# DarlingHang/st-nerf

Measured on NVIDIA H100. Metric: rays/sec, higher is better.
Workload: dtype f32 via fp16x3 split products (wgmma), f32 accumulate

## Files before the change

st-nerf_b200/csrc/mlp_tc.cu:

```cuda
#include <cuda_fp16.h>
#include <string.h>
#include <type_traits>
#include <vector>
#include "mlp_tc.cuh"
#include "resample.cuh"

namespace stnerf {

namespace {

constexpr int TILE_M = 128;
constexpr int ABLOCK = 16384;
constexpr int STAGE_BYTES = 16384;
constexpr int NTHREADS = 384;
constexpr int MATH_WG0 = 1, N_MATH_WARPS = 8;
constexpr int MAX_STAGE = 8;
constexpr int REGS_WG0 = 56, REGS_MATH = 224;
static_assert(128 * REGS_WG0 + 256 * REGS_MATH <= 384 * 168, "register file");
constexpr int BAR_WFULL = 0, BAR_WEMPTY = 8, BAR_RAWFULL = 16, BAR_RAWEMPTY = 18;
constexpr int MISC_ROWS = 256;
constexpr int MISC_PART = MISC_ROWS + 128 * 24;
constexpr int MISC_CDF = MISC_PART + 2048;
constexpr int MISC_TOTAL = MISC_CDF + 512;

__device__ __forceinline__ uint32_t smem_u32(const void* p) { return (uint32_t)__cvta_generic_to_shared(p); }

__device__ __forceinline__ void mbar_init(uint32_t bar, uint32_t count) {
  asm volatile("mbarrier.init.shared::cta.b64 [%0], %1;" ::"r"(bar), "r"(count) : "memory");
}
__device__ __forceinline__ void mbar_arrive(uint32_t bar) {
  asm volatile("mbarrier.arrive.shared::cta.b64 _, [%0];" ::"r"(bar) : "memory");
}
__device__ __forceinline__ void mbar_arrive_if(uint32_t bar, bool pred) {
  asm volatile("{\n\t.reg .pred p;\n\tsetp.ne.b32 p, %1, 0;\n\t@p mbarrier.arrive.shared::cta.b64 _, [%0];\n\t}" ::"r"(bar), "r"((uint32_t)pred)
               : "memory");
}
__device__ __forceinline__ void mbar_expect_tx(uint32_t bar, uint32_t bytes) {
  asm volatile("mbarrier.arrive.expect_tx.shared::cta.b64 _, [%0], %1;" ::"r"(bar), "r"(bytes) : "memory");
}
__device__ __forceinline__ void mbar_wait(uint32_t bar, uint32_t parity) {
  asm volatile(
      "{\n\t.reg .pred p;\n\t.reg .u32 c;\n\t"
      "mov.u32 c, 0;\n"
      "WAIT_%=:\n\t"
      "mbarrier.try_wait.parity.shared::cta.b64 p, [%0], %1;\n\t"
      "@p bra.uni DONE_%=;\n\t"
      "add.u32 c, c, 1;\n\t"
      "setp.gt.u32 p, c, 67108864;\n\t"
      "@p trap;\n\t"
      "bra.uni WAIT_%=;\n"
      "DONE_%=:\n\t}" ::"r"(bar), "r"(parity)
      : "memory");
}
__device__ __forceinline__ void bulk_g2s(uint32_t dst, const void* src, uint32_t bytes, uint32_t bar) {
  asm volatile("cp.async.bulk.shared::cluster.global.mbarrier::complete_tx::bytes [%0], [%1], %2, [%3];" ::"r"(dst),
               "l"(src), "r"(bytes), "r"(bar)
               : "memory");
}
__device__ __forceinline__ void fence_proxy_async() { asm volatile("fence.proxy.async.shared::cta;" ::: "memory"); }
template <int R>
__device__ __forceinline__ void setmaxnreg_dec() { asm volatile("setmaxnreg.dec.sync.aligned.u32 %0;" ::"n"(R)); }
template <int R>
__device__ __forceinline__ void setmaxnreg_inc() { asm volatile("setmaxnreg.inc.sync.aligned.u32 %0;" ::"n"(R)); }
__device__ __forceinline__ void wg_bar_sync(int wg) { asm volatile("bar.sync %0, 128;" ::"r"(1 + wg) : "memory"); }

__device__ __forceinline__ void load_stage_elect(uint32_t dst, const void* src, uint32_t bytes, uint32_t bar) {
  asm volatile(
      "{\n\t.reg .pred pe;\n\t"
      "elect.sync _|pe, 0xffffffff;\n\t"
      "@pe mbarrier.arrive.expect_tx.shared::cta.b64 _, [%3], %2;\n\t"
      "@pe cp.async.bulk.shared::cluster.global.mbarrier::complete_tx::bytes [%0], [%1], %2, [%3];\n\t}" ::"r"(dst),
      "l"(src), "r"(bytes), "r"(bar)
      : "memory");
}

__device__ __forceinline__ uint64_t desc_sw128(uint32_t saddr) {
  return (uint64_t)((saddr >> 4) & 0x3FFF) | ((uint64_t)1 << 16) | ((uint64_t)(1024 >> 4) << 32) | ((uint64_t)1 << 62);
}
__device__ __forceinline__ uint64_t desc_sw64(uint32_t saddr) {
  return (uint64_t)((saddr >> 4) & 0x3FFF) | ((uint64_t)1 << 16) | ((uint64_t)(512 >> 4) << 32) | ((uint64_t)2 << 62);
}
__device__ __forceinline__ void wgmma_fence() { asm volatile("wgmma.fence.sync.aligned;" ::: "memory"); }
__device__ __forceinline__ void wgmma_commit() { asm volatile("wgmma.commit_group.sync.aligned;" ::: "memory"); }
template <int N>
__device__ __forceinline__ void wgmma_wait() { asm volatile("wgmma.wait_group.sync.aligned %0;" ::"n"(N) : "memory"); }
template <int R>
__device__ __forceinline__ void acc_fence(float (&d)[128]) {
#pragma unroll
  for (int i = 0; i < R; ++i) asm volatile("" : "+f"(d[i])::"memory");
}

#define WGMMA_D_LO "%0, %1, %2, %3, %4, %5, %6, %7, %8, %9, %10, %11, %12, %13, %14, %15, %16, %17, %18, %19, %20, %21, %22, %23, %24, %25, %26, %27, %28, %29, %30, %31, %32, %33, %34, %35, %36, %37, %38, %39, %40, %41, %42, %43, %44, %45, %46, %47, %48, %49, %50, %51, %52, %53, %54, %55, %56, %57, %58, %59, %60, %61, %62, %63"
#define WGMMA_D_HI "%64, %65, %66, %67, %68, %69, %70, %71, %72, %73, %74, %75, %76, %77, %78, %79, %80, %81, %82, %83, %84, %85, %86, %87, %88, %89, %90, %91, %92, %93, %94, %95, %96, %97, %98, %99, %100, %101, %102, %103, %104, %105, %106, %107, %108, %109, %110, %111, %112, %113, %114, %115, %116, %117, %118, %119, %120, %121, %122, %123, %124, %125, %126, %127"
#define WGMMA_OPS_LO(d) \
    "+f"(d[0]), "+f"(d[1]), "+f"(d[2]), "+f"(d[3]), "+f"(d[4]), "+f"(d[5]), "+f"(d[6]), "+f"(d[7]), \
    "+f"(d[8]), "+f"(d[9]), "+f"(d[10]), "+f"(d[11]), "+f"(d[12]), "+f"(d[13]), "+f"(d[14]), "+f"(d[15]), \
    "+f"(d[16]), "+f"(d[17]), "+f"(d[18]), "+f"(d[19]), "+f"(d[20]), "+f"(d[21]), "+f"(d[22]), "+f"(d[23]), \
    "+f"(d[24]), "+f"(d[25]), "+f"(d[26]), "+f"(d[27]), "+f"(d[28]), "+f"(d[29]), "+f"(d[30]), "+f"(d[31]), \
    "+f"(d[32]), "+f"(d[33]), "+f"(d[34]), "+f"(d[35]), "+f"(d[36]), "+f"(d[37]), "+f"(d[38]), "+f"(d[39]), \
    "+f"(d[40]), "+f"(d[41]), "+f"(d[42]), "+f"(d[43]), "+f"(d[44]), "+f"(d[45]), "+f"(d[46]), "+f"(d[47]), \
    "+f"(d[48]), "+f"(d[49]), "+f"(d[50]), "+f"(d[51]), "+f"(d[52]), "+f"(d[53]), "+f"(d[54]), "+f"(d[55]), \
    "+f"(d[56]), "+f"(d[57]), "+f"(d[58]), "+f"(d[59]), "+f"(d[60]), "+f"(d[61]), "+f"(d[62]), "+f"(d[63])
#define WGMMA_OPS_HI(d) \
    "+f"(d[64]), "+f"(d[65]), "+f"(d[66]), "+f"(d[67]), "+f"(d[68]), "+f"(d[69]), "+f"(d[70]), "+f"(d[71]), \
    "+f"(d[72]), "+f"(d[73]), "+f"(d[74]), "+f"(d[75]), "+f"(d[76]), "+f"(d[77]), "+f"(d[78]), "+f"(d[79]), \
    "+f"(d[80]), "+f"(d[81]), "+f"(d[82]), "+f"(d[83]), "+f"(d[84]), "+f"(d[85]), "+f"(d[86]), "+f"(d[87]), \
    "+f"(d[88]), "+f"(d[89]), "+f"(d[90]), "+f"(d[91]), "+f"(d[92]), "+f"(d[93]), "+f"(d[94]), "+f"(d[95]), \
    "+f"(d[96]), "+f"(d[97]), "+f"(d[98]), "+f"(d[99]), "+f"(d[100]), "+f"(d[101]), "+f"(d[102]), "+f"(d[103]), \
    "+f"(d[104]), "+f"(d[105]), "+f"(d[106]), "+f"(d[107]), "+f"(d[108]), "+f"(d[109]), "+f"(d[110]), "+f"(d[111]), \
    "+f"(d[112]), "+f"(d[113]), "+f"(d[114]), "+f"(d[115]), "+f"(d[116]), "+f"(d[117]), "+f"(d[118]), "+f"(d[119]), \
    "+f"(d[120]), "+f"(d[121]), "+f"(d[122]), "+f"(d[123]), "+f"(d[124]), "+f"(d[125]), "+f"(d[126]), "+f"(d[127])

__device__ __forceinline__ void wgmma_n256(float (&d)[128], uint64_t da, uint64_t db) {
  asm volatile(
      "{\n\t.reg .pred p;\n\tsetp.ne.b32 p, %130, 0;\n\t"
      "wgmma.mma_async.sync.aligned.m64n256k16.f32.f16.f16 "
      "{" WGMMA_D_LO ", " WGMMA_D_HI "}, %128, %129, p, 1, 1, 0, 0;\n\t}"
      : WGMMA_OPS_LO(d), WGMMA_OPS_HI(d)
      : "l"(da), "l"(db), "r"(1));
}
__device__ __forceinline__ void wgmma_n128(float (&d)[128], uint64_t da, uint64_t db) {
  asm volatile(
      "{\n\t.reg .pred p;\n\tsetp.ne.b32 p, %66, 0;\n\t"
      "wgmma.mma_async.sync.aligned.m64n128k16.f32.f16.f16 "
      "{" WGMMA_D_LO "}, %64, %65, p, 1, 1, 0, 0;\n\t}"
      : WGMMA_OPS_LO(d)
      : "l"(da), "l"(db), "r"(1));
}
__device__ __forceinline__ void wgmma_n256_rs(float (&d)[128], const uint32_t* a, uint64_t db) {
  asm volatile(
      "{\n\t.reg .pred p;\n\tsetp.ne.b32 p, %133, 0;\n\t"
      "wgmma.mma_async.sync.aligned.m64n256k16.f32.f16.f16 "
      "{" WGMMA_D_LO ", " WGMMA_D_HI "}, {%128, %129, %130, %131}, %132, p, 1, 1, 0;\n\t}"
      : WGMMA_OPS_LO(d), WGMMA_OPS_HI(d)
      : "r"(a[0]), "r"(a[1]), "r"(a[2]), "r"(a[3]), "l"(db), "r"(1));
}
__device__ __forceinline__ void wgmma_n128_rs(float (&d)[128], const uint32_t* a, uint64_t db) {
  asm volatile(
      "{\n\t.reg .pred p;\n\tsetp.ne.b32 p, %69, 0;\n\t"
      "wgmma.mma_async.sync.aligned.m64n128k16.f32.f16.f16 "
      "{" WGMMA_D_LO "}, {%64, %65, %66, %67}, %68, p, 1, 1, 0;\n\t}"
      : WGMMA_OPS_LO(d)
      : "r"(a[0]), "r"(a[1]), "r"(a[2]), "r"(a[3]), "l"(db), "r"(1));
}

template <int N>
__device__ __forceinline__ void wgmma_k16(float (&d)[128], uint64_t da, uint64_t db) {
  if (N == 256) wgmma_n256(d, da, db);
  else wgmma_n128(d, da, db);
}
template <int N>
__device__ __forceinline__ void wgmma_k16_rs(float (&d)[128], const uint32_t* a, uint64_t db) {
  if (N == 256) wgmma_n256_rs(d, a, db);
  else wgmma_n128_rs(d, a, db);
}

__device__ __forceinline__ uint32_t pack_f16x2(float a, float b) {
  uint32_t r;
  asm("cvt.rn.satfinite.f16x2.f32 %0, %1, %2;" : "=r"(r) : "f"(b), "f"(a));
  return r;
}
__device__ __forceinline__ float2 unpack_f16x2(uint32_t p) {
  return __half22float2(*reinterpret_cast<const __half2*>(&p));
}

__host__ __device__ inline uint32_t sw128_offset(int row, int col) {
  return (uint32_t)((row >> 3) * 1024 + (row & 7) * 128 + ((((col >> 3) ^ (row & 7)) & 7) << 4) + ((col & 7) << 1));
}
__host__ __device__ inline uint32_t sw64_offset(int row, int col) {
  return (uint32_t)((row >> 3) * 512 + (row & 7) * 64 + ((((col >> 3) ^ ((row >> 1) & 3)) & 3) << 4) + ((col & 7) << 1));
}

enum { NET_SPACE = 0, NET_MOTION = 1 };

template <int NET> struct Sched;
template <> struct Sched<NET_SPACE> {
  static constexpr int N_LAYERS = 8;
  static constexpr bool lo_in_regs = true;
  static constexpr int act_base = 0, enc_base = 4 * ABLOCK;
  static constexpr int ENC_LO_STRIDE = ABLOCK;
  static constexpr int n_stage = 7, stage_bytes = STAGE_BYTES;
  static constexpr int ring_base = 6 * ABLOCK, misc_base = ring_base + n_stage * stage_bytes, smem_total = misc_base + MISC_TOTAL;
  static_assert(smem_total <= 232448, "shared memory budget (227 KB per CTA)");
  __host__ __device__ static constexpr int n_out(int l) { return l == 7 ? 128 : 256; }
  __host__ __device__ static constexpr int act_chunks(int l) { return l == 0 ? 0 : 4; }
  __host__ __device__ static constexpr int enc_chunks(int l) { return (l == 0 || l == 4) ? 1 : 0; }
  __host__ __device__ static constexpr bool enc_first(int l) { return l == 4; }
};
template <> struct Sched<NET_MOTION> {
  static constexpr int N_LAYERS = 5;
  static constexpr bool lo_in_regs = false;
  static constexpr int act_base = 0, enc_base = 0;
  static constexpr int LO_STRIDE = 2 * ABLOCK;
  static constexpr int ENC_LO_STRIDE = 2 * ABLOCK;
  static constexpr int n_stage = 8, stage_bytes = 8192;
  static constexpr int ring_base = 4 * ABLOCK, misc_base = ring_base + n_stage * stage_bytes, smem_total = misc_base + MISC_TOTAL;
  __host__ __device__ static constexpr int n_out(int) { return 128; }
  __host__ __device__ static constexpr int act_chunks(int l) { return l == 0 ? 0 : 2; }
  __host__ __device__ static constexpr int enc_chunks(int l) { return l == 0 ? 2 : 0; }
  __host__ __device__ static constexpr bool enc_first(int) { return false; }
};
static_assert(Sched<NET_SPACE>::n_stage <= MAX_STAGE && Sched<NET_MOTION>::n_stage <= MAX_STAGE, "barrier slots");

enum { A_HI = 0, A_LO = 1, A_HI_LO = 2 };
template <int A>
struct WStep {
  static constexpr int a = A;
  uint32_t offset;
  uint32_t sub;
};
template <int NET>
struct WSched {
  using S = Sched<NET>;
  __host__ __device__ static constexpr int n_chunks(int l) { return S::act_chunks(l) + S::enc_chunks(l); }
  __host__ __device__ static constexpr uint32_t stage_bytes(int l) { return (uint32_t)S::n_out(l) * 64; }
  __host__ __device__ static constexpr size_t layer_bytes(int l) { return (size_t)n_chunks(l) * 2  * 2  * stage_bytes(l); }
  __host__ __device__ static constexpr int chunk_at(int l, int c) {
    return S::enc_first(l) ? (c == 0 ? S::act_chunks(l) : c - 1) : c;
  }
  static constexpr bool enc_first_valid() {
    for (int l = 0; l < S::N_LAYERS; ++l)
      if (S::enc_first(l) && (S::act_chunks(l) == 0 || S::enc_chunks(l) == 0)) return false;
    return true;
  }
  static_assert(enc_first_valid(), "enc_first(l) needs activation chunks and an encoding chunk to reorder");
  template <bool LOFIRST, class C, class F>
  __device__ __forceinline__ static void for_each_step(int l, bool split, C&& chunk, F&& f) {
    const int nact = S::act_chunks(l), nch = nact + S::enc_chunks(l);
    const uint32_t bytes = stage_bytes(l);
    auto at = [&](const auto& a, int c, uint32_t sub, uint32_t lo_stage, auto op) {
      f(a, WStep<decltype(op)::value>{(2 * (2 * (uint32_t)c + sub) + lo_stage) * bytes, sub});
    };
    using HI = std::integral_constant<int, A_HI>;
    using LO = std::integral_constant<int, A_LO>;
    using HI_LO = std::integral_constant<int, A_HI_LO>;
    if (!LOFIRST || !split) {
      for (int c = 0; c < nch; ++c) {
        const auto a = chunk(chunk_at(l, c));
        for (uint32_t sub = 0; sub < 2; ++sub) {
          if (split) { at(a, c, sub, 1u, HI()); at(a, c, sub, 0u, HI_LO()); }
          else at(a, c, sub, 0u, HI());
        }
      }
    } else {
      for (int c = 0; c < nch; ++c) {
        const auto a = chunk(chunk_at(l, c));
        for (uint32_t sub = 0; sub < 2; ++sub) { at(a, c, sub, 1u, HI()); at(a, c, sub, 0u, LO()); }
      }
      for (int c = 0; c < nch; ++c) {
        const auto a = chunk(chunk_at(l, c));
        for (uint32_t sub = 0; sub < 2; ++sub) at(a, c, sub, 0u, HI());
      }
    }
  }
};

template <int NET>
__host__ __device__ constexpr size_t stream_bytes_per_tile() {
  size_t n = 0;
  for (int l = 0; l < Sched<NET>::N_LAYERS; ++l) n += WSched<NET>::layer_bytes(l);
  return n;
}

struct TcParams {
  FuseCoarse fuse;
  PointSrc src;
  const uint8_t* wstream;
  const float* aux;
  const float* cbuf;
  int exact;
  int single_last;
  int lo_first;
  float* raw;
  float* rgb_out;
  float* sigma_out;
  float* xyz_out;
  float* flow_out;
  const int* lerp_flag;
  int lerp_force;
};

constexpr int AUX_BIAS = 0, AUX_WSIG = 8 * 256, AUX_BSIG = AUX_WSIG + 256, AUX_WOUT = AUX_BSIG + 4,
              AUX_BOUT = AUX_WOUT + 3 * 128, AUX_FLOATS = AUX_BOUT + 4;


struct Pt { float x, y, z, tm; int out_index; int cidx; };

__device__ __forceinline__ Pt fetch_pt(const PointSrc& s, long long p, long long n_points) {
  Pt q;
  q.x = q.y = q.z = q.tm = 0.f;
  q.out_index = -1;
  q.cidx = 0;
  if (p >= n_points) return q;
  if (s.mode == SRC_EXPLICIT) {
    const float* pp = s.pos + p * s.pos_stride;
    q.x = pp[0]; q.y = pp[1]; q.z = pp[2];
    if (s.times) q.tm = s.times[p * s.time_stride];
    q.out_index = (int)p;
    q.cidx = (int)p;
    return q;
  }
  const long long slot = p / s.S;
  const int k = (int)(p - slot * s.S);
  const long long ray = s.hit ? (long long)s.hit[slot] : slot;
  const float* rp = s.rays + ray * s.ray_stride;
  q.tm = rp[6 + s.layer];
  q.out_index = (int)(ray * s.S + k);
  q.cidx = (int)slot;
  if (s.mode == SRC_XYZ) {
    q.x = s.pos[3 * p]; q.y = s.pos[3 * p + 1]; q.z = s.pos[3 * p + 2];
    return q;
  }
  if (s.mode == SRC_XYZ_MAP) {
    const int m = s.src_map[ray * s.S + k];
    const float* pp = (m < s.n_first) ? s.pos + 3 * (slot * s.n_first + m) : s.pos2 + 3 * (slot * (s.S - s.n_first) + (m - s.n_first));
    q.x = pp[0]; q.y = pp[1]; q.z = pp[2];
    return q;
  }
  const float tt = s.t[ray * s.S + k];
  float v[3] = {__fadd_rn(__fmul_rn(tt, rp[3]), rp[0]), __fadd_rn(__fmul_rn(tt, rp[4]), rp[1]),
                __fadd_rn(__fmul_rn(tt, rp[5]), rp[2])};
#pragma unroll
  for (int a = 0; a < 3; ++a) {
    if (s.shift_on) v[a] = __fsub_rn(v[a], s.shift[a]);
    if (s.scale_on) v[a] = __fadd_rn(__fdiv_rn(__fsub_rn(v[a], s.pivot[a]), s.scale), s.pivot[a]);
  }
  q.x = v[0]; q.y = v[1]; q.z = v[2];
  return q;
}

struct SinCos3 { float s0, s1, s2, c0, c1, c2; };
struct SinCos4 { float s0, s1, s2, s3, c0, c1, c2, c3; };
__device__ __noinline__ SinCos3 sincos_full3(float x0, float x1, float x2) {
  SinCos3 r;
  sincosf(x0, &r.s0, &r.c0); sincosf(x1, &r.s1, &r.c1); sincosf(x2, &r.s2, &r.c2);
  return r;
}
__device__ __noinline__ SinCos4 sincos_full4(float x0, float x1, float x2, float x3) {
  SinCos4 r;
  sincosf(x0, &r.s0, &r.c0); sincosf(x1, &r.s1, &r.c1); sincosf(x2, &r.s2, &r.c2); sincosf(x3, &r.s3, &r.c3);
  return r;
}

template <int NV>
__device__ __forceinline__ void store_row_split(uint8_t* hi_blk, int lo_stride, int row, int col0, const float (&v)[NV],
                                                bool exact) {
#pragma unroll
  for (int g = 0; g < NV / 8; ++g) {
    uint32_t hp[4], lp[4];
#pragma unroll
    for (int e = 0; e < 4; ++e) {
      const float a = v[g * 8 + 2 * e], b = v[g * 8 + 2 * e + 1];
      hp[e] = pack_f16x2(a, b);
      const float2 hf = unpack_f16x2(hp[e]);
      lp[e] = pack_f16x2(a - hf.x, b - hf.y);
    }
    const uint32_t off = sw128_offset(row, col0 + g * 8);
    *reinterpret_cast<uint4*>(hi_blk + off) = make_uint4(hp[0], hp[1], hp[2], hp[3]);
    if (exact) *reinterpret_cast<uint4*>(hi_blk + lo_stride + off) = make_uint4(lp[0], lp[1], lp[2], lp[3]);
  }
}

template <int half, int piece>
__device__ __forceinline__ void encode_space_piece(uint8_t* smem, const Pt& pt, int row, bool exact, float (&carry)[2]) {
  using S = Sched<NET_SPACE>;
  uint8_t* enc = smem + S::enc_base;
  const float xs[3] = {pt.x, pt.y, pt.z};
  float v[16];
  auto trig = [&](int f, float* dst) {
    const float fr = (float)(1 << f);
    const SinCos3 q = sincos_full3(xs[0] * fr, xs[1] * fr, xs[2] * fr);
    dst[0] = q.s0; dst[1] = q.s1; dst[2] = q.s2; dst[3] = q.c0; dst[4] = q.c1; dst[5] = q.c2;
  };
  if (piece == 0) {
    float t3[6];
    trig(5 * half + 0, v); trig(5 * half + 1, v + 6); trig(5 * half + 2, t3);
    v[12] = t3[0]; v[13] = t3[1]; v[14] = t3[2]; v[15] = t3[3];
    carry[0] = t3[4]; carry[1] = t3[5];
  } else {
    v[0] = carry[0]; v[1] = carry[1];
    trig(5 * half + 3, v + 2); trig(5 * half + 4, v + 8);
    v[14] = half == 0 ? xs[0] : xs[2];
    v[15] = half == 0 ? xs[1] : 0.f;
  }
  store_row_split<16>(enc, S::ENC_LO_STRIDE, row, half * 32 + piece * 16, v, exact);
}

template <int half, int piece>
__device__ __forceinline__ void encode_motion_piece(uint8_t* smem, const Pt& pt, int row, bool exact, bool lerp) {
  using S = Sched<NET_MOTION>;
  uint8_t* enc = smem + S::enc_base + half * ABLOCK;
  const float lo_t = floorf(pt.tm), wgt = pt.tm - lo_t, omw = 1.0f - wgt;
  const float in4[4] = {pt.x, pt.y, pt.z, pt.tm};
  auto trig = [&](int f, float* dst) {
    const float fr = (float)(1 << f);
    if (!lerp) {
      const SinCos4 q = sincos_full4(in4[0] * fr, in4[1] * fr, in4[2] * fr, in4[3] * fr);
      dst[0] = q.s0; dst[1] = q.s1; dst[2] = q.s2; dst[3] = q.s3; dst[4] = q.c0; dst[5] = q.c1; dst[6] = q.c2; dst[7] = q.c3;
    } else {
      const SinCos4 q = sincos_full4(in4[0] * fr, in4[1] * fr, in4[2] * fr, lo_t * fr);
      const SinCos3 q1 = sincos_full3((lo_t + 1.0f) * fr, 0.f, 0.f);
      const float s0[4] = {q.s0, q.s1, q.s2, q.s3}, c0[4] = {q.c0, q.c1, q.c2, q.c3};
      const float s1[4] = {q.s0, q.s1, q.s2, q1.s0}, c1[4] = {q.c0, q.c1, q.c2, q1.c0};
#pragma unroll
      for (int d = 0; d < 4; ++d) {
        dst[d] = __fadd_rn(__fmul_rn(omw, s0[d]), __fmul_rn(wgt, s1[d]));
        dst[4 + d] = __fadd_rn(__fmul_rn(omw, c0[d]), __fmul_rn(wgt, c1[d]));
      }
    }
  };
  float v[16];
  trig(5 * half + 2 * piece, v);
  if (piece < 2) {
    trig(5 * half + 2 * piece + 1, v + 8);
  } else {
#pragma unroll
    for (int d = 0; d < 4; ++d) {
      float a = 0.f;
      if (half == 0) {
        a = in4[d];
        if (lerp) {
          const float lo = d < 3 ? in4[d] : lo_t, hi = d < 3 ? in4[d] : lo_t + 1.0f;
          a = __fadd_rn(__fmul_rn(omw, lo), __fmul_rn(wgt, hi));
        }
      }
      v[8 + d] = a; v[12 + d] = 0.f;
    }
  }
  store_row_split<16>(enc, S::ENC_LO_STRIDE, row, piece * 16, v, exact);
}

template <int NET, int piece>
__device__ __forceinline__ void encode_piece(uint8_t* smem, const Pt& pt, int row, int half, bool exact, bool lerp,
                                             float (&carry)[2]) {
  if (NET == NET_SPACE) {
    if (half == 0) encode_space_piece<0, piece < 2 ? piece : 1>(smem, pt, row, exact, carry);
    else encode_space_piece<1, piece < 2 ? piece : 1>(smem, pt, row, exact, carry);
  } else {
    if (half == 0) encode_motion_piece<0, piece>(smem, pt, row, exact, lerp);
    else encode_motion_piece<1, piece>(smem, pt, row, exact, lerp);
  }
}

template <int NZ>
__device__ __noinline__ void fused_composite_loop(const TcParams& P, const float* rows, float* cdf, uint32_t bar_full, uint32_t bar_empty,
                                                  long long n_tiles, int j, int lane) {
  const FuseCoarse& F = P.fuse;
  const PointSrc& src = P.src;
  const long long n_slots = src.count ? (long long)(*src.count) : src.n_slots;
  const int n1 = 64, n2 = F.n2;
  uint32_t n = 0;
  for (long long tile = blockIdx.x; tile < n_tiles; tile += gridDim.x, ++n) {
    mbar_wait(bar_full, n & 1);
    const long long slot = tile * 2 + j;
    if (slot < n_slots) {
      const long long ray = src.hit ? (long long)src.hit[slot] : slot;
      const float* tp = src.t + ray * n1;
      const float4* rp = reinterpret_cast<const float4*>(rows) + j * 64;
      float t[2], sg[2];
#pragma unroll
      for (int s = 0; s < 2; ++s) {
        const int k = s * 32 + lane;
        const float tk = __ldg(tp + k);
        float v = rp[k].w;
        if (F.is_bkgd) {
          if (tk < F.near_plane) v = 0.0f;
        } else {
          if (tk < 0.0f) v = 0.0f;
          if (F.apply_thr && v < F.thr) v = 0.0f;
        }
        t[s] = tk;
        sg[s] = v;
      }
      const float* up = F.u ? F.u + ray * n2 : nullptr;
      const uint64_t seed = F.seed;
      const uint32_t stream = 64u + (uint32_t)F.layer;
      const unsigned long long gid = F.idmap(F.ray_base + ray);
      rs::LayerOut lo;
      rs::composite_resample_ray<2, NZ>(
          t, sg, n1, n2, F.boarder,
          [rp, lane](int s) {
            const float4 v = rp[s * 32 + lane];
            return make_float3(__fdiv_rn(1.0f, __fadd_rn(1.0f, expf(-v.x))), __fdiv_rn(1.0f, __fadd_rn(1.0f, expf(-v.y))),
                               __fdiv_rn(1.0f, __fadd_rn(1.0f, expf(-v.z))));
          },
          [up, seed, stream, gid](int jj) { return up ? up[jj] : philox_uniform(seed, stream, gid, (uint32_t)jj); },
          cdf, F.t_fine + ray * (n1 + n2), lane, lo, F.z_new ? F.z_new + ray * n2 : nullptr,
          F.z_new ? F.src_map + ray * (n1 + n2) : nullptr);
      if (F.img && lane < 5) {
        const long long rg = F.ray_base + ray;
        const float v = lane == 0 ? lo.pix[0] : lane == 1 ? lo.pix[1] : lane == 2 ? lo.pix[2] : lane == 3 ? lo.pix[3] : lo.pix[4];
        if (F.pixels) F.img[rg * 5 + lane] = v;
        else if (lane < 3) F.img[rg * 3 + lane] = v;
        else F.img[(long long)lane * F.n_total + rg] = v;
      }
    }
    __syncwarp();
    if (lane == 0) mbar_arrive(bar_empty);
  }
}

template <int NET, int N, bool LOFIRST>
__device__ __forceinline__ void mma_layer(float (&acc)[128], const uint32_t (&alo)[64], int l, bool sp, uint32_t sbase,
                                          uint32_t a_row, uint32_t bars, uint32_t& cnt, int lane) {
  using S = Sched<NET>;
  using W = WSched<NET>;
  constexpr uint32_t NST = S::n_stage;
#pragma unroll
  for (int i = 0; i < N / 2; ++i) acc[i] = 0.f;
  acc_fence<N / 2>(acc);
  wgmma_fence();
  const int nact = S::act_chunks(l);
  int pend = -1;
  auto release = [&](int s) {
    __syncwarp();
    mbar_arrive_if(bars + 8u * (uint32_t)(BAR_WEMPTY + s), lane == 0);
  };
  auto a_block = [&](int ch) {
    uint32_t hi, lo = 0;
    int z = -1;
    if (ch < nact) {
      hi = sbase + S::act_base + ch * ABLOCK + a_row;
      if constexpr (S::lo_in_regs) z = ch;
      else lo = hi + S::LO_STRIDE;
    } else {
      hi = sbase + S::enc_base + (ch - nact) * ABLOCK + a_row;
      lo = hi + S::ENC_LO_STRIDE;
    }
    return make_int3((int)hi, (int)lo, z);
  };
  W::template for_each_step<LOFIRST>(l, sp, a_block, [&](const int3& a, auto st) {
    const uint32_t hi = (uint32_t)a.x + 64u * st.sub, lo = (uint32_t)a.y + 64u * st.sub;
    const uint32_t s = cnt % NST, n = cnt / NST;
    mbar_wait(bars + 8u * (BAR_WFULL + s), n & 1);
    const uint32_t w = sbase + S::ring_base + s * S::stage_bytes;
    auto mma_lo = [&]() {
      if (S::lo_in_regs && a.z >= 0) {
        const int q = 2 * a.z + (int)st.sub;
#pragma unroll
        for (int i = 0; i < 8; ++i)
          if (q == i) {
#pragma unroll
            for (int ks = 0; ks < 2; ++ks) wgmma_k16_rs<N>(acc, &alo[8 * i + 4 * ks], desc_sw64(w + ks * 32));
          }
      } else {
#pragma unroll
        for (int ks = 0; ks < 2; ++ks) wgmma_k16<N>(acc, desc_sw128(lo + ks * 32), desc_sw64(w + ks * 32));
      }
    };
    if constexpr (decltype(st)::a == A_LO) {
      mma_lo();
    } else {
#pragma unroll
      for (int ks = 0; ks < 2; ++ks) wgmma_k16<N>(acc, desc_sw128(hi + ks * 32), desc_sw64(w + ks * 32));
      if constexpr (decltype(st)::a == A_HI_LO) mma_lo();
    }
    wgmma_commit();
    wgmma_wait<1>();
    if (pend >= 0) release(pend);
    pend = (int)s;
    ++cnt;
  });
  wgmma_wait<0>();
  acc_fence<N / 2>(acc);
  release(pend);
}

template <int NET, int N, bool SIGMA>
__device__ __forceinline__ void epi_hidden(const float (&acc)[128], const float* __restrict__ bias, const float* __restrict__ wsig,
                                           uint8_t* smem, int r0, int cq, bool lo_too, float& sig0, float& sig1,
                                           uint32_t (&alo)[64]) {
  using S = Sched<NET>;
#pragma unroll
  for (int j = 0; j < N / 8; ++j) {
    const int col = 8 * j + cq;
    const float2 b = __ldg(reinterpret_cast<const float2*>(bias + col));
    const float v00 = fmaxf(acc[4 * j] + b.x, 0.f), v01 = fmaxf(acc[4 * j + 1] + b.y, 0.f);
    const float v10 = fmaxf(acc[4 * j + 2] + b.x, 0.f), v11 = fmaxf(acc[4 * j + 3] + b.y, 0.f);
    if (SIGMA) {
      const float2 w = __ldg(reinterpret_cast<const float2*>(wsig + col));
      sig0 = fmaf(v00, w.x, sig0); sig0 = fmaf(v01, w.y, sig0);
      sig1 = fmaf(v10, w.x, sig1); sig1 = fmaf(v11, w.y, sig1);
    }
    uint8_t* blk = smem + S::act_base + (col >> 6) * ABLOCK;
    const uint32_t o0 = sw128_offset(r0, col & 63), o1 = sw128_offset(r0 + 8, col & 63);
    const uint32_t h0 = pack_f16x2(v00, v01), h1 = pack_f16x2(v10, v11);
    *reinterpret_cast<uint32_t*>(blk + o0) = h0;
    *reinterpret_cast<uint32_t*>(blk + o1) = h1;
    const float2 f0 = unpack_f16x2(h0), f1 = unpack_f16x2(h1);
    const uint32_t l0 = pack_f16x2(v00 - f0.x, v01 - f0.y), l1 = pack_f16x2(v10 - f1.x, v11 - f1.y);
    if constexpr (S::lo_in_regs) {
      alo[2 * j] = l0;
      alo[2 * j + 1] = l1;
    } else if (lo_too) {
      *reinterpret_cast<uint32_t*>(blk + S::LO_STRIDE + o0) = l0;
      *reinterpret_cast<uint32_t*>(blk + S::LO_STRIDE + o1) = l1;
    }
  }
}

__device__ __forceinline__ float quad_sum(float v) {
  v += __shfl_xor_sync(0xffffffffu, v, 1);
  v += __shfl_xor_sync(0xffffffffu, v, 2);
  return v;
}

template <int NET, bool LOFIRST>
__global__ void __launch_bounds__(NTHREADS, 1) mlp_tc_kernel(const __grid_constant__ TcParams P) {
  using S = Sched<NET>;
  extern __shared__ __align__(1024) uint8_t smem[];
  const uint32_t sbase = smem_u32(smem);
  if ((sbase & 1023u) != 0) {
    if (threadIdx.x == 0) printf("stnerf mlp_tc: dynamic shared memory base %u is not 1024-byte aligned\n", sbase);
    __trap();
  }
  const uint32_t bars = sbase + S::misc_base;
  auto BAR = [bars](int i) { return bars + 8u * (uint32_t)i; };
  Pt* s_rows = reinterpret_cast<Pt*>(smem + S::misc_base + MISC_ROWS);
  float* s_part = reinterpret_cast<float*>(smem + S::misc_base + MISC_PART);

  const int tid = threadIdx.x, lane = tid & 31;
  const int warp = __shfl_sync(0xffffffffu, tid >> 5, 0);
  const int wgi = __shfl_sync(0xffffffffu, tid >> 7, 0);
  const bool exact = P.exact != 0;
  const bool single_last = P.single_last != 0;
  auto split = [&](int l) { return exact && !(single_last && l == S::N_LAYERS - 1); };
  const long long n_points = src_num_points(P.src);
  const long long n_tiles = (n_points + TILE_M - 1) / TILE_M;
  constexpr uint32_t NST = S::n_stage;
  if (tid == 0) {
    for (int i = 0; i < MAX_STAGE; ++i) { mbar_init(BAR(BAR_WFULL + i), 1); mbar_init(BAR(BAR_WEMPTY + i), N_MATH_WARPS); }
    for (int j = 0; j < 2; ++j) {
      mbar_init(BAR(BAR_RAWFULL + j), 4);
      mbar_init(BAR(BAR_RAWEMPTY + j), 1);
    }
    asm volatile("fence.mbarrier_init.release.cluster;" ::: "memory");
  }
  __syncthreads();

  if (wgi < MATH_WG0) {
    if constexpr (S::lo_in_regs) setmaxnreg_dec<REGS_WG0>();
    if (warp == 0) {
      using W = WSched<NET>;
      uint32_t cnt = 0;
      for (long long tile = blockIdx.x; tile < n_tiles; tile += gridDim.x) {
        const uint8_t* layer = P.wstream;
        for (int l = 0; l < S::N_LAYERS; ++l) {
          W::template for_each_step<LOFIRST>(l, split(l), [](int) { return 0; }, [&](int, auto st) {
            const uint32_t s = cnt % NST, n = cnt / NST;
            mbar_wait(BAR(BAR_WEMPTY + s), (n & 1) ^ 1);
            load_stage_elect(sbase + S::ring_base + s * S::stage_bytes, layer + st.offset, W::stage_bytes(l), BAR(BAR_WFULL + s));
            ++cnt;
          });
          layer += W::layer_bytes(l);
        }
      }
    } else if (NET == NET_SPACE && (warp == 2 || warp == 3)) {
      if (P.fuse.on) {
        const int j = warp - 2;
        float* cdf = reinterpret_cast<float*>(smem + S::misc_base + MISC_CDF) + j * 64;
        if (P.fuse.n2 <= 128)
          fused_composite_loop<4>(P, s_part, cdf, BAR(BAR_RAWFULL + j), BAR(BAR_RAWEMPTY + j), n_tiles, j, lane);
        else
          fused_composite_loop<8>(P, s_part, cdf, BAR(BAR_RAWFULL + j), BAR(BAR_RAWEMPTY + j), n_tiles, j, lane);
      }
    }
  } else {
    if constexpr (S::lo_in_regs) setmaxnreg_inc<REGS_MATH>();
    const int wg = wgi - MATH_WG0;
    const int wt = tid & 127;
    const int erow = wg * 64 + (wt & 63), ehalf = wt >> 6;
    const int r0 = wg * 64 + (wt >> 5) * 16 + (lane >> 2);
    const int cq = 2 * (lane & 3);
    const uint32_t a_row = (uint32_t)wg * 8u * 1024u;
    const float* bias_all = P.aux + AUX_BIAS;
    const bool lerp = (NET == NET_MOTION) && (P.lerp_force >= 0 ? (P.lerp_force != 0) : (P.lerp_flag && *P.lerp_flag != 0));
    const bool fused = (NET == NET_SPACE) && P.fuse.on;
    uint32_t cnt = 0, tile_no = 0;
    float acc[128];
    uint32_t alo[64];
#pragma unroll
    for (int i = 0; i < 64; ++i) alo[i] = 0u;
    for (long long tile = blockIdx.x; tile < n_tiles; tile += gridDim.x, ++tile_no) {
      wg_bar_sync(wg);
      const Pt cur = fetch_pt(P.src, tile * TILE_M + erow, n_points);
      if (ehalf == 0) s_rows[erow] = cur;
      float carry[2] = {0.f, 0.f};
      if (NET == NET_MOTION) {
        uint8_t* enc = smem + S::enc_base + ehalf * ABLOCK;
        for (int c = (ehalf == 0 ? 48 : 40); c < 64; c += 8) {
          const uint32_t off = sw128_offset(erow, c);
          *reinterpret_cast<uint4*>(enc + off) = make_uint4(0, 0, 0, 0);
          *reinterpret_cast<uint4*>(enc + S::ENC_LO_STRIDE + off) = make_uint4(0, 0, 0, 0);
        }
      }
      encode_piece<NET, 0>(smem, cur, erow, ehalf, exact, lerp, carry);
      encode_piece<NET, 1>(smem, cur, erow, ehalf, exact, lerp, carry);
      if (NET == NET_MOTION) encode_piece<NET, 2>(smem, cur, erow, ehalf, exact, lerp, carry);
      float sig0 = 0.f, sig1 = 0.f;
      for (int l = 0; l < S::N_LAYERS; ++l) {
        fence_proxy_async();
        wg_bar_sync(wg);
        const bool last = (l == S::N_LAYERS - 1);
        if (!last) {
          mma_layer<NET, (NET == NET_SPACE ? 256 : 128), LOFIRST>(acc, alo, l, split(l), sbase, a_row, bars, cnt, lane);
          if (NET == NET_SPACE && l == 6)
            epi_hidden<NET, 256, true>(acc, bias_all + l * 256, P.aux + AUX_WSIG, smem, r0, cq, split(l + 1), sig0, sig1, alo);
          else
            epi_hidden<NET, (NET == NET_SPACE ? 256 : 128), false>(acc, bias_all + l * 256, nullptr, smem, r0, cq, split(l + 1), sig0,
                                                                  sig1, alo);
          continue;
        }
        mma_layer<NET, 128, LOFIRST>(acc, alo, l, split(l), sbase, a_row, bars, cnt, lane);
        const Pt p0 = s_rows[r0], p1 = s_rows[r0 + 8];
        const float* b0 = (NET == NET_SPACE) ? (P.cbuf + (size_t)p0.cidx * 128) : bias_all + l * 256;
        const float* b1 = (NET == NET_SPACE) ? (P.cbuf + (size_t)p1.cidx * 128) : bias_all + l * 256;
        float d0[3] = {0.f, 0.f, 0.f}, d1[3] = {0.f, 0.f, 0.f};
#pragma unroll
        for (int j = 0; j < 16; ++j) {
          const int col = 8 * j + cq;
          const float2 ba = __ldg(reinterpret_cast<const float2*>(b0 + col));
          const float2 bb = __ldg(reinterpret_cast<const float2*>(b1 + col));
          const float v00 = fmaxf(acc[4 * j] + ba.x, 0.f), v01 = fmaxf(acc[4 * j + 1] + ba.y, 0.f);
          const float v10 = fmaxf(acc[4 * j + 2] + bb.x, 0.f), v11 = fmaxf(acc[4 * j + 3] + bb.y, 0.f);
#pragma unroll
          for (int o = 0; o < 3; ++o) {
            const float2 w = __ldg(reinterpret_cast<const float2*>(P.aux + AUX_WOUT + o * 128 + col));
            d0[o] = fmaf(v00, w.x, d0[o]); d0[o] = fmaf(v01, w.y, d0[o]);
            d1[o] = fmaf(v10, w.x, d1[o]); d1[o] = fmaf(v11, w.y, d1[o]);
          }
        }
#pragma unroll
        for (int o = 0; o < 3; ++o) { d0[o] = quad_sum(d0[o]) + P.aux[AUX_BOUT + o]; d1[o] = quad_sum(d1[o]) + P.aux[AUX_BOUT + o]; }
        if (NET == NET_SPACE) { sig0 = quad_sum(sig0) + P.aux[AUX_BSIG]; sig1 = quad_sum(sig1) + P.aux[AUX_BSIG]; }
        if (fused) {
          if (tile_no > 0) mbar_wait(BAR(BAR_RAWEMPTY + wg), (tile_no - 1) & 1);
          if ((lane & 3) == 0) {
            reinterpret_cast<float4*>(s_part)[r0] = make_float4(d0[0], d0[1], d0[2], sig0);
            reinterpret_cast<float4*>(s_part)[r0 + 8] = make_float4(d1[0], d1[1], d1[2], sig1);
          }
          __syncwarp();
          if (lane == 0) mbar_arrive(BAR(BAR_RAWFULL + wg));
        }
        if ((lane & 3) == 0) {
#pragma unroll
          for (int h = 0; h < 2; ++h) {
            const Pt& p = h ? p1 : p0;
            const float* o = h ? d1 : d0;
            const float sg = h ? sig1 : sig0;
            if (p.out_index < 0) continue;
            const int oi = p.out_index;
            if (NET == NET_SPACE) {
              if (P.raw) reinterpret_cast<float4*>(P.raw)[oi] = make_float4(o[0], o[1], o[2], sg);
              if (P.rgb_out) { P.rgb_out[3 * (size_t)oi] = o[0]; P.rgb_out[3 * (size_t)oi + 1] = o[1]; P.rgb_out[3 * (size_t)oi + 2] = o[2]; }
              if (P.sigma_out) P.sigma_out[oi] = sg;
            } else {
              const long long pidx = tile * TILE_M + r0 + 8 * h;
              if (P.flow_out) { P.flow_out[3 * pidx] = o[0]; P.flow_out[3 * pidx + 1] = o[1]; P.flow_out[3 * pidx + 2] = o[2]; }
              if (P.xyz_out) {
                P.xyz_out[3 * pidx] = __fadd_rn(p.x, o[0]);
                P.xyz_out[3 * pidx + 1] = __fadd_rn(p.y, o[1]);
                P.xyz_out[3 * pidx + 2] = __fadd_rn(p.z, o[2]);
              }
            }
          }
        }
      }
    }
  }
}

constexpr int HB_SLOTS = 8;
__global__ void __launch_bounds__(128) head_bias_kernel(PointSrc src, const float* __restrict__ w_tail ,
                                                        const float* __restrict__ b1, int use_time,
                                                        float* __restrict__ cbuf) {
  __shared__ float s_enc[HB_SLOTS][48];
  const long long n_slots = src.count ? (long long)(*src.count) : src.n_slots;
  const int nk = PE_DIR + (use_time ? PE_TIME : 0);
  const int tid = threadIdx.x;
  float w[48];
#pragma unroll
  for (int k = 0; k < 48; ++k) w[k] = (k < nk) ? __ldg(w_tail + k * 128 + tid) : 0.f;
  const float bias = __ldg(b1 + tid);
  for (long long s0 = (long long)blockIdx.x * HB_SLOTS; s0 < n_slots; s0 += (long long)gridDim.x * HB_SLOTS) {
    __syncthreads();
    for (int e = tid; e < HB_SLOTS * 48; e += 128) {
      const int sl = e / 48, j = e - sl * 48;
      const long long slot = s0 + sl;
      float v = 0.f;
      if (slot < n_slots && j < nk) {
        float d[3], tm;
        if (src.mode == SRC_EXPLICIT) {
          d[0] = src.dirs[3 * slot]; d[1] = src.dirs[3 * slot + 1]; d[2] = src.dirs[3 * slot + 2];
          tm = src.times ? src.times[slot * src.time_stride] : 0.f;
        } else {
          const long long ray = src.hit ? (long long)src.hit[slot] : slot;
          const float* rp = src.rays + ray * src.ray_stride;
          d[0] = rp[3]; d[1] = rp[4]; d[2] = rp[5];
          tm = rp[6 + src.layer];
        }
        if (j < PE_DIR) {
          if (j < 3) v = d[j];
          else {
            const int r = j - 3, f = r / 6, m = r - 6 * f;
            const float a = d[m % 3] * (float)(1 << f);
            v = (m < 3) ? sinf(a) : cosf(a);
          }
        } else {
          const int r = j - PE_DIR;
          if (r == 0) v = tm;
          else {
            const int f = (r - 1) >> 1;
            const float a = tm * (float)(1 << f);
            v = ((r - 1) & 1) ? cosf(a) : sinf(a);
          }
        }
        v = fmaxf(v, 0.f);
      }
      s_enc[sl][j] = v;
    }
    __syncthreads();
#pragma unroll
    for (int sl = 0; sl < HB_SLOTS; ++sl) {
      const long long slot = s0 + sl;
      if (slot >= n_slots) break;
      float acc = bias;
#pragma unroll
      for (int k = 0; k < 48; ++k) acc = fmaf(w[k], s_enc[sl][k], acc);
      cbuf[slot * 128 + tid] = acc;
    }
  }
}

__global__ void __launch_bounds__(256, 1) wgmma_selftest_kernel(const float* __restrict__ A, const uint8_t* __restrict__ Bstages,
                                                               float* __restrict__ D, int reps) {
  extern __shared__ __align__(1024) uint8_t smem[];
  const uint32_t sbase = smem_u32(smem);
  const uint32_t bar = sbase + ABLOCK + 2 * STAGE_BYTES;
  const int tid = threadIdx.x, wg = tid >> 7, wt = tid & 127, lane = tid & 31;
  if ((sbase & 1023u) != 0) __trap();
  if (tid == 0) {
    mbar_init(bar, 1);
    asm volatile("fence.mbarrier_init.release.cluster;" ::: "memory");
  }
  if (tid < 128) {
    for (int c0 = 0; c0 < 64; c0 += 32) {
      float v[32];
      for (int i = 0; i < 32; ++i) v[i] = A[tid * 64 + c0 + i];
      store_row_split<32>(smem, 0, tid, c0, v, false);
    }
  }
  fence_proxy_async();
  __syncthreads();
  if (tid == 0) {
    mbar_expect_tx(bar, 2 * STAGE_BYTES);
    bulk_g2s(sbase + ABLOCK, Bstages, 2 * STAGE_BYTES, bar);
  }
  mbar_wait(bar, 0);
  float acc[128];
#pragma unroll
  for (int i = 0; i < 128; ++i) acc[i] = 0.f;
  acc_fence<128>(acc);
  wgmma_fence();
  for (int rep = 0; rep < reps; ++rep) {
#pragma unroll
    for (int sub = 0; sub < 2; ++sub)
#pragma unroll
// ... 273 lines not shown
```

Measured before the change: 750,800.

## Move positional encoding to producer warps with double-buffered mbarrier handoff

```diff
diff --git a/st-nerf_b200/csrc/mlp_tc.cu b/st-nerf_b200/csrc/mlp_tc.cu
--- a/st-nerf_b200/csrc/mlp_tc.cu
+++ b/st-nerf_b200/csrc/mlp_tc.cu
@@ -17,9 +17,9 @@
 constexpr int MAX_STAGE = 8;
 constexpr int REGS_WG0 = 56, REGS_MATH = 224;
 static_assert(128 * REGS_WG0 + 256 * REGS_MATH <= 384 * 168, "register file");
-constexpr int BAR_WFULL = 0, BAR_WEMPTY = 8, BAR_RAWFULL = 16, BAR_RAWEMPTY = 18;
+constexpr int BAR_WFULL = 0, BAR_WEMPTY = 8, BAR_RAWFULL = 16, BAR_RAWEMPTY = 18, BAR_ENCFULL = 20, BAR_ENCEMPTY = 21;
 constexpr int MISC_ROWS = 256;
-constexpr int MISC_PART = MISC_ROWS + 128 * 24;
+constexpr int MISC_PART = MISC_ROWS + 2 * 128 * 24;
 constexpr int MISC_CDF = MISC_PART + 2048;
 constexpr int MISC_TOTAL = MISC_CDF + 512;
 
@@ -186,19 +186,22 @@
   __host__ __device__ static constexpr int act_chunks(int l) { return l == 0 ? 0 : 4; }
   __host__ __device__ static constexpr int enc_chunks(int l) { return (l == 0 || l == 4) ? 1 : 0; }
   __host__ __device__ static constexpr bool enc_first(int l) { return l == 4; }
+  static constexpr int enc_last_layer = 4;
 };
 template <> struct Sched<NET_MOTION> {
   static constexpr int N_LAYERS = 5;
   static constexpr bool lo_in_regs = false;
-  static constexpr int act_base = 0, enc_base = 0;
+  static constexpr int act_base = 0, enc_base = 4 * ABLOCK;
   static constexpr int LO_STRIDE = 2 * ABLOCK;
   static constexpr int ENC_LO_STRIDE = 2 * ABLOCK;
   static constexpr int n_stage = 8, stage_bytes = 8192;
-  static constexpr int ring_base = 4 * ABLOCK, misc_base = ring_base + n_stage * stage_bytes, smem_total = misc_base + MISC_TOTAL;
+  static constexpr int ring_base = 8 * ABLOCK, misc_base = ring_base + n_stage * stage_bytes, smem_total = misc_base + MISC_TOTAL;
+  static_assert(smem_total <= 232448, "shared memory budget (227 KB per CTA)");
   __host__ __device__ static constexpr int n_out(int) { return 128; }
   __host__ __device__ static constexpr int act_chunks(int l) { return l == 0 ? 0 : 2; }
   __host__ __device__ static constexpr int enc_chunks(int l) { return l == 0 ? 2 : 0; }
   __host__ __device__ static constexpr bool enc_first(int) { return false; }
+  static constexpr int enc_last_layer = 0;
 };
 static_assert(Sched<NET_SPACE>::n_stage <= MAX_STAGE && Sched<NET_MOTION>::n_stage <= MAX_STAGE, "barrier slots");
 
@@ -224,6 +227,12 @@
     return true;
   }
   static_assert(enc_first_valid(), "enc_first(l) needs activation chunks and an encoding chunk to reorder");
+  template <bool LOFIRST>
+  __host__ __device__ static constexpr int last_enc_step(int l, bool split) {
+    const int nch = n_chunks(l), pos = S::enc_first(l) ? 0 : nch - 1;
+    if (LOFIRST && split) return 4 * nch + 2 * (pos + 1) - 1;
+    return (split ? 4 : 2) * (pos + 1) - 1;
+  }
   template <bool LOFIRST, class C, class F>
   __device__ __forceinline__ static void for_each_step(int l, bool split, C&& chunk, F&& f) {
     const int nact = S::act_chunks(l), nch = nact + S::enc_chunks(l);
@@ -329,19 +338,6 @@
   return q;
 }
 
-struct SinCos3 { float s0, s1, s2, c0, c1, c2; };
-struct SinCos4 { float s0, s1, s2, s3, c0, c1, c2, c3; };
-__device__ __noinline__ SinCos3 sincos_full3(float x0, float x1, float x2) {
-  SinCos3 r;
-  sincosf(x0, &r.s0, &r.c0); sincosf(x1, &r.s1, &r.c1); sincosf(x2, &r.s2, &r.c2);
-  return r;
-}
-__device__ __noinline__ SinCos4 sincos_full4(float x0, float x1, float x2, float x3) {
-  SinCos4 r;
-  sincosf(x0, &r.s0, &r.c0); sincosf(x1, &r.s1, &r.c1); sincosf(x2, &r.s2, &r.c2); sincosf(x3, &r.s3, &r.c3);
-  return r;
-}
-
 template <int NV>
 __device__ __forceinline__ void store_row_split(uint8_t* hi_blk, int lo_stride, int row, int col0, const float (&v)[NV],
                                                 bool exact) {
@@ -361,84 +357,71 @@
   }
 }
 
-template <int half, int piece>
-__device__ __forceinline__ void encode_space_piece(uint8_t* smem, const Pt& pt, int row, bool exact, float (&carry)[2]) {
-  using S = Sched<NET_SPACE>;
+template <int NV>
+__device__ __forceinline__ void store_pairs_split(uint8_t* hi_blk, int lo_stride, int row, int col0, const float (&v)[NV],
+                                                  bool exact) {
+#pragma unroll
+  for (int e = 0; e < NV / 2; ++e) {
+    const uint32_t hp = pack_f16x2(v[2 * e], v[2 * e + 1]);
+    const float2 hf = unpack_f16x2(hp);
+    const uint32_t off = sw128_offset(row, col0 + 2 * e);
+    *reinterpret_cast<uint32_t*>(hi_blk + off) = hp;
+    if (exact) *reinterpret_cast<uint32_t*>(hi_blk + lo_stride + off) = pack_f16x2(v[2 * e] - hf.x, v[2 * e + 1] - hf.y);
+  }
+}
+
+template <int NET>
+__device__ __forceinline__ void encode_row(uint8_t* smem, const Pt& pt, int row, bool exact, bool lerp) {
+  using S = Sched<NET>;
   uint8_t* enc = smem + S::enc_base;
-  const float xs[3] = {pt.x, pt.y, pt.z};
-  float v[16];
-  auto trig = [&](int f, float* dst) {
-    const float fr = (float)(1 << f);
-    const SinCos3 q = sincos_full3(xs[0] * fr, xs[1] * fr, xs[2] * fr);
-    dst[0] = q.s0; dst[1] = q.s1; dst[2] = q.s2; dst[3] = q.c0; dst[4] = q.c1; dst[5] = q.c2;
-  };
-  if (piece == 0) {
-    float t3[6];
-    trig(5 * half + 0, v); trig(5 * half + 1, v + 6); trig(5 * half + 2, t3);
-    v[12] = t3[0]; v[13] = t3[1]; v[14] = t3[2]; v[15] = t3[3];
-    carry[0] = t3[4]; carry[1] = t3[5];
+  if constexpr (NET == NET_SPACE) {
+#pragma unroll 1
+    for (int f = 0; f < 10; ++f) {
+      const float fr = (float)(1 << f);
+      float v[6];
+      sincosf(pt.x * fr, &v[0], &v[3]); sincosf(pt.y * fr, &v[1], &v[4]); sincosf(pt.z * fr, &v[2], &v[5]);
+      store_pairs_split<6>(enc, S::ENC_LO_STRIDE, row, 32 * (f / 5) + 6 * (f % 5), v, exact);
+    }
+    const float xy[2] = {pt.x, pt.y}, z0[2] = {pt.z, 0.f};
+    store_pairs_split<2>(enc, S::ENC_LO_STRIDE, row, 30, xy, exact);
+    store_pairs_split<2>(enc, S::ENC_LO_STRIDE, row, 62, z0, exact);
   } else {
-    v[0] = carry[0]; v[1] = carry[1];
-    trig(5 * half + 3, v + 2); trig(5 * half + 4, v + 8);
-    v[14] = half == 0 ? xs[0] : xs[2];
-    v[15] = half == 0 ? xs[1] : 0.f;
-  }
-  store_row_split<16>(enc, S::ENC_LO_STRIDE, row, half * 32 + piece * 16, v, exact);
-}
-
-template <int half, int piece>
-__device__ __forceinline__ void encode_motion_piece(uint8_t* smem, const Pt& pt, int row, bool exact, bool lerp) {
-  using S = Sched<NET_MOTION>;
-  uint8_t* enc = smem + S::enc_base + half * ABLOCK;
-  const float lo_t = floorf(pt.tm), wgt = pt.tm - lo_t, omw = 1.0f - wgt;
-  const float in4[4] = {pt.x, pt.y, pt.z, pt.tm};
-  auto trig = [&](int f, float* dst) {
-    const float fr = (float)(1 << f);
-    if (!lerp) {
-      const SinCos4 q = sincos_full4(in4[0] * fr, in4[1] * fr, in4[2] * fr, in4[3] * fr);
-      dst[0] = q.s0; dst[1] = q.s1; dst[2] = q.s2; dst[3] = q.s3; dst[4] = q.c0; dst[5] = q.c1; dst[6] = q.c2; dst[7] = q.c3;
-    } else {
-      const SinCos4 q = sincos_full4(in4[0] * fr, in4[1] * fr, in4[2] * fr, lo_t * fr);
-      const SinCos3 q1 = sincos_full3((lo_t + 1.0f) * fr, 0.f, 0.f);
-      const float s0[4] = {q.s0, q.s1, q.s2, q.s3}, c0[4] = {q.c0, q.c1, q.c2, q.c3};
-      const float s1[4] = {q.s0, q.s1, q.s2, q1.s0}, c1[4] = {q.c0, q.c1, q.c2, q1.c0};
-#pragma unroll
-      for (int d = 0; d < 4; ++d) {
-        dst[d] = __fadd_rn(__fmul_rn(omw, s0[d]), __fmul_rn(wgt, s1[d]));
-        dst[4 + d] = __fadd_rn(__fmul_rn(omw, c0[d]), __fmul_rn(wgt, c1[d]));
-      }
-    }
-  };
-  float v[16];
-  trig(5 * half + 2 * piece, v);
-  if (piece < 2) {
-    trig(5 * half + 2 * piece + 1, v + 8);
-  } else {
+    const float lo_t = floorf(pt.tm), wgt = pt.tm - lo_t, omw = 1.0f - wgt;
+    const float in4[4] = {pt.x, pt.y, pt.z, pt.tm};
+#pragma unroll 1
+    for (int f = 0; f < 10; ++f) {
+      const float fr = (float)(1 << f);
+      float v[8];
+      if (!lerp) {
+#pragma unroll
+        for (int d = 0; d < 4; ++d) sincosf(in4[d] * fr, &v[d], &v[4 + d]);
+      } else {
+        float s0[4], c0[4], s1[4], c1[4];
+#pragma unroll
+        for (int d = 0; d < 3; ++d) sincosf(in4[d] * fr, &s0[d], &c0[d]);
+        sincosf(lo_t * fr, &s0[3], &c0[3]);
+        sincosf((lo_t + 1.0f) * fr, &s1[3], &c1[3]);
+#pragma unroll
+        for (int d = 0; d < 3; ++d) { s1[d] = s0[d]; c1[d] = c0[d]; }
+#pragma unroll
+        for (int d = 0; d < 4; ++d) {
+          v[d] = __fadd_rn(__fmul_rn(omw, s0[d]), __fmul_rn(wgt, s1[d]));
+          v[4 + d] = __fadd_rn(__fmul_rn(omw, c0[d]), __fmul_rn(wgt, c1[d]));
+        }
+      }
+      store_row_split<8>(enc + (f / 5) * ABLOCK, S::ENC_LO_STRIDE, row, 8 * (f % 5), v, exact);
+    }
+    float raw[8];
 #pragma unroll
     for (int d = 0; d < 4; ++d) {
-      float a = 0.f;
-      if (half == 0) {
-        a = in4[d];
-        if (lerp) {
-          const float lo = d < 3 ? in4[d] : lo_t, hi = d < 3 ? in4[d] : lo_t + 1.0f;
-          a = __fadd_rn(__fmul_rn(omw, lo), __fmul_rn(wgt, hi));
-        }
-      }
-      v[8 + d] = a; v[12 + d] = 0.f;
-    }
-  }
-  store_row_split<16>(enc, S::ENC_LO_STRIDE, row, piece * 16, v, exact);
-}
-
-template <int NET, int piece>
-__device__ __forceinline__ void encode_piece(uint8_t* smem, const Pt& pt, int row, int half, bool exact, bool lerp,
-                                             float (&carry)[2]) {
-  if (NET == NET_SPACE) {
-    if (half == 0) encode_space_piece<0, piece < 2 ? piece : 1>(smem, pt, row, exact, carry);
-    else encode_space_piece<1, piece < 2 ? piece : 1>(smem, pt, row, exact, carry);
-  } else {
-    if (half == 0) encode_motion_piece<0, piece>(smem, pt, row, exact, lerp);
-    else encode_motion_piece<1, piece>(smem, pt, row, exact, lerp);
+      float a = in4[d];
+      if (lerp) {
+        const float lo = d < 3 ? in4[d] : lo_t, hi = d < 3 ? in4[d] : lo_t + 1.0f;
+        a = __fadd_rn(__fmul_rn(omw, lo), __fmul_rn(wgt, hi));
+      }
+      raw[d] = a; raw[4 + d] = 0.f;
+    }
+    store_row_split<8>(enc, S::ENC_LO_STRIDE, row, 40, raw, exact);
   }
 }
 
@@ -502,7 +485,7 @@
 
 template <int NET, int N, bool LOFIRST>
 __device__ __forceinline__ void mma_layer(float (&acc)[128], const uint32_t (&alo)[64], int l, bool sp, uint32_t sbase,
-                                          uint32_t a_row, uint32_t bars, uint32_t& cnt, int lane) {
+                                          uint32_t a_row, uint32_t bars, uint32_t& cnt, int lane, int enc_last) {
   using S = Sched<NET>;
   using W = WSched<NET>;
   constexpr uint32_t NST = S::n_stage;
@@ -511,10 +494,11 @@
   acc_fence<N / 2>(acc);
   wgmma_fence();
   const int nact = S::act_chunks(l);
-  int pend = -1;
-  auto release = [&](int s) {
+  int pend = -1, step = 0;
+  auto release = [&](int s, int k) {
     __syncwarp();
     mbar_arrive_if(bars + 8u * (uint32_t)(BAR_WEMPTY + s), lane == 0);
+    if (k == enc_last) mbar_arrive_if(bars + 8u * (uint32_t)BAR_ENCEMPTY, lane == 0);
   };
   auto a_block = [&](int ch) {
     uint32_t hi, lo = 0;
@@ -557,13 +541,14 @@
     }
     wgmma_commit();
     wgmma_wait<1>();
-    if (pend >= 0) release(pend);
+    if (pend >= 0) release(pend, step - 1);
     pend = (int)s;
     ++cnt;
+    ++step;
   });
   wgmma_wait<0>();
   acc_fence<N / 2>(acc);
-  release(pend);
+  release(pend, step - 1);
 }
 
 template <int NET, int N, bool SIGMA>
@@ -628,12 +613,15 @@
   const long long n_points = src_num_points(P.src);
   const long long n_tiles = (n_points + TILE_M - 1) / TILE_M;
   constexpr uint32_t NST = S::n_stage;
+  const int n_loaders = (NET == NET_SPACE && P.fuse.on) ? 1 : 2;
   if (tid == 0) {
     for (int i = 0; i < MAX_STAGE; ++i) { mbar_init(BAR(BAR_WFULL + i), 1); mbar_init(BAR(BAR_WEMPTY + i), N_MATH_WARPS); }
     for (int j = 0; j < 2; ++j) {
       mbar_init(BAR(BAR_RAWFULL + j), 4);
       mbar_init(BAR(BAR_RAWEMPTY + j), 1);
     }
+    mbar_init(BAR(BAR_ENCFULL), n_loaders);
+    mbar_init(BAR(BAR_ENCEMPTY), N_MATH_WARPS);
     asm volatile("fence.mbarrier_init.release.cluster;" ::: "memory");
   }
   __syncthreads();
@@ -655,6 +643,34 @@
           layer += W::layer_bytes(l);
         }
       }
+    } else if (warp <= n_loaders) {
+      const bool lerp = (NET == NET_MOTION) && (P.lerp_force >= 0 ? (P.lerp_force != 0) : (P.lerp_flag && *P.lerp_flag != 0));
+      const int per = TILE_M / 32 / n_loaders, row0 = (warp - 1) * per * 32 + lane;
+      if (NET == NET_MOTION && warp == 1) {
+        for (int r = lane; r < TILE_M; r += 32)
+          for (int b = 0; b < 2; ++b)
+            for (int c = b == 0 ? 48 : 40; c < 64; c += 8) {
+              uint8_t* p = smem + S::enc_base + b * ABLOCK + sw128_offset(r, c);
+              *reinterpret_cast<uint4*>(p) = make_uint4(0, 0, 0, 0);
+              *reinterpret_cast<uint4*>(p + S::ENC_LO_STRIDE) = make_uint4(0, 0, 0, 0);
+            }
+      }
+      uint32_t k = 0;
+      for (long long tile = blockIdx.x; tile < n_tiles; tile += gridDim.x, ++k) {
+        Pt q[TILE_M / 32];
+#pragma unroll
+        for (int i = 0; i < TILE_M / 32; ++i)
+          if (i < per) q[i] = fetch_pt(P.src, tile * TILE_M + row0 + 32 * i, n_points);
+        mbar_wait(BAR(BAR_ENCEMPTY), (k & 1) ^ 1);
+        Pt* rows = s_rows + (k & 1) * TILE_M;
+#pragma unroll
+        for (int i = 0; i < TILE_M / 32; ++i)
+          if (i < per) rows[row0 + 32 * i] = q[i];
+        for (int i = 0; i < per; ++i) encode_row<NET>(smem, rows[row0 + 32 * i], row0 + 32 * i, exact, lerp);
+        fence_proxy_async();
+        __syncwarp();
+        if (lane == 0) mbar_arrive(BAR(BAR_ENCFULL));
+      }
     } else if (NET == NET_SPACE && (warp == 2 || warp == 3)) {
       if (P.fuse.on) {
         const int j = warp - 2;
@@ -667,14 +683,13 @@
     }
   } else {
     if constexpr (S::lo_in_regs) setmaxnreg_inc<REGS_MATH>();
+    using W = WSched<NET>;
     const int wg = wgi - MATH_WG0;
     const int wt = tid & 127;
-    const int erow = wg * 64 + (wt & 63), ehalf = wt >> 6;
     const int r0 = wg * 64 + (wt >> 5) * 16 + (lane >> 2);
     const int cq = 2 * (lane & 3);
     const uint32_t a_row = (uint32_t)wg * 8u * 1024u;
     const float* bias_all = P.aux + AUX_BIAS;
-    const bool lerp = (NET == NET_MOTION) && (P.lerp_force >= 0 ? (P.lerp_force != 0) : (P.lerp_flag && *P.lerp_flag != 0));
     const bool fused = (NET == NET_SPACE) && P.fuse.on;
     uint32_t cnt = 0, tile_no = 0;
     float acc[128];
@@ -682,28 +697,17 @@
 #pragma unroll
     for (int i = 0; i < 64; ++i) alo[i] = 0u;
     for (long long tile = blockIdx.x; tile < n_tiles; tile += gridDim.x, ++tile_no) {
-      wg_bar_sync(wg);
-      const Pt cur = fetch_pt(P.src, tile * TILE_M + erow, n_points);
-      if (ehalf == 0) s_rows[erow] = cur;
-      float carry[2] = {0.f, 0.f};
-      if (NET == NET_MOTION) {
-        uint8_t* enc = smem + S::enc_base + ehalf * ABLOCK;
-        for (int c = (ehalf == 0 ? 48 : 40); c < 64; c += 8) {
-          const uint32_t off = sw128_offset(erow, c);
-          *reinterpret_cast<uint4*>(enc + off) = make_uint4(0, 0, 0, 0);
-          *reinterpret_cast<uint4*>(enc + S::ENC_LO_STRIDE + off) = make_uint4(0, 0, 0, 0);
-        }
-      }
-      encode_piece<NET, 0>(smem, cur, erow, ehalf, exact, lerp, carry);
-      encode_piece<NET, 1>(smem, cur, erow, ehalf, exact, lerp, carry);
-      if (NET == NET_MOTION) encode_piece<NET, 2>(smem, cur, erow, ehalf, exact, lerp, carry);
+      mbar_wait(BAR(BAR_ENCFULL), tile_no & 1);
+      const Pt* rows = s_rows + (tile_no & 1) * TILE_M;
       float sig0 = 0.f, sig1 = 0.f;
       for (int l = 0; l < S::N_LAYERS; ++l) {
         fence_proxy_async();
         wg_bar_sync(wg);
         const bool last = (l == S::N_LAYERS - 1);
+        const int enc_last = l == S::enc_last_layer ? W::template last_enc_step<LOFIRST>(l, split(l)) : -1;
         if (!last) {
-          mma_layer<NET, (NET == NET_SPACE ? 256 : 128), LOFIRST>(acc, alo, l, split(l), sbase, a_row, bars, cnt, lane);
+          mma_layer<NET, (NET == NET_SPACE ? 256 : 128), LOFIRST>(acc, alo, l, split(l), sbase, a_row, bars, cnt, lane,
+                                                                  enc_last);
           if (NET == NET_SPACE && l == 6)
             epi_hidden<NET, 256, true>(acc, bias_all + l * 256, P.aux + AUX_WSIG, smem, r0, cq, split(l + 1), sig0, sig1, alo);
           else
@@ -711,8 +715,8 @@
                                                                   sig1, alo);
           continue;
         }
-        mma_layer<NET, 128, LOFIRST>(acc, alo, l, split(l), sbase, a_row, bars, cnt, lane);
-        const Pt p0 = s_rows[r0], p1 = s_rows[r0 + 8];
+        mma_layer<NET, 128, LOFIRST>(acc, alo, l, split(l), sbase, a_row, bars, cnt, lane, enc_last);
+        const Pt p0 = rows[r0], p1 = rows[r0 + 8];
         const float* b0 = (NET == NET_SPACE) ? (P.cbuf + (size_t)p0.cidx * 128) : bias_all + l * 256;
         const float* b1 = (NET == NET_SPACE) ? (P.cbuf + (size_t)p1.cidx * 128) : bias_all + l * 256;
         float d0[3] = {0.f, 0.f, 0.f}, d1[3] = {0.f, 0.f, 0.f};
```

New measurement: 761,700, median of 6. 1.01x the previous value.
